# sjulier/Refactored_ORB_SLAM2

Measured on AMD Instinct MI355X. Metric: frames/s (extract+match) at KITTI 1241×376, 2000 feat; 1/2/4/8 GPU + CPU ref, higher is better.
Workload: dtype u8; 1 GPU; kitti_stereo_1241x376_2000feat_8lvl: 2x ORBextractor + ComputeStereoMatches + SearchByProjection(cur,last); parallelism=frame-shard x1, collective=none, driver=torch, queries=one pass: orbfe_track_queries_stereo_device

## Files before the change

refactored_orb_slam2_amd/csrc/match_kernels.hip:

```cpp
#include <string.h>
#include <atomic>
#include <mutex>

#include "match_internal.h"

#define WAVE 64

__device__ __forceinline__ int hamming256(const uint4 a0, const uint4 a1, const uint4 b0, const uint4 b1) {
  return __popc(a0.x ^ b0.x) + __popc(a0.y ^ b0.y) + __popc(a0.z ^ b0.z) + __popc(a0.w ^ b0.w) +
         __popc(a1.x ^ b1.x) + __popc(a1.y ^ b1.y) + __popc(a1.z ^ b1.z) + __popc(a1.w ^ b1.w);
}
__device__ __forceinline__ void load_desc(const uint8_t* p, uint4& d0, uint4& d1) {
  const uint4* q = reinterpret_cast<const uint4*>(p);
  d0 = q[0];
  d1 = q[1];
}
__device__ __forceinline__ void load_desc4(const uint8_t* p, uint4& d0, uint4& d1) {
  const uint32_t* q = reinterpret_cast<const uint32_t*>(p);
  d0 = make_uint4(q[0], q[1], q[2], q[3]);
  d1 = make_uint4(q[4], q[5], q[6], q[7]);
}

__device__ __forceinline__ unsigned wave_min_u32(unsigned v) {
#define ORBFE_MIN_STEP(ctrl, rmask) v = min(v, (unsigned)__builtin_amdgcn_update_dpp((int)0xffffffff, (int)v, ctrl, rmask, 0xf, false))
// ... 837 lines not shown
  for (int i = lane; i < pr.countB; i += WAVE)
    taken[i] = (uint8_t)((P.sequential && __hip_atomic_load(&P.matchB[P.idxB[pr.startB + i]], __ATOMIC_RELAXED, __HIP_MEMORY_SCOPE_AGENT) >= 0) ||
                         (P.validB && !P.validB[P.idxB[pr.startB + i]]));
  __syncthreads();
  for (int iKF = 0; iKF < pr.countA; iKF++) {
    const int realIdxKF = P.idxA[pr.startA + iKF];
    if (!P.validA[realIdxKF]) continue;
    uint4 a0, a1;
    load_desc(P.descA + (size_t)realIdxKF * 32, a0, a1);
    int bestd = 256, bestj = -1, second = 256;
    for (int iF = lane; iF < pr.countB; iF += WAVE) {
      if (taken[iF]) continue;
      const int realIdxF = P.idxB[pr.startB + iF];
      uint4 b0, b1;
      load_desc(P.descB + (size_t)realIdxF * 32, b0, b1);
      const int d = hamming256(a0, a1, b0, b1);
      if (d < bestd) { second = bestd; bestd = d; bestj = iF; }
      else if (d < second) second = d;
    }
    const unsigned key = bestj >= 0 ? (((unsigned)bestd << 16) | (unsigned)bestj) : 0xFFFFFFFFu;
    const unsigned b = wave_min_u32(key);
    if (b != 0xFFFFFFFFu) {
      const unsigned other = (key == b) ? 0xFFFFFFFFu : key;
      int s2 = min(second, other != 0xFFFFFFFFu ? (int)(other >> 16) : 256);
#pragma unroll
      for (int d = 32; d >= 1; d >>= 1) s2 = min(s2, __shfl_xor(s2, d, WAVE));
      const int bestDist1 = (int)(b >> 16), bestF = (int)(b & 0xffff);
      if ((P.kf_mode ? bestDist1 < ORBFE_TH_LOW : bestDist1 <= ORBFE_TH_LOW) && (float)bestDist1 < P.nnratio * (float)s2) {
        if (lane == 0) {
          const int realIdxF = P.idxB[pr.startB + bestF];
          __hip_atomic_store(&P.matchB[realIdxF], realIdxKF, __ATOMIC_RELAXED, __HIP_MEMORY_SCOPE_AGENT);
          if (P.kf_mode) P.matchA[realIdxKF] = realIdxF;
          taken[bestF] = 1;
          if (P.sequential)
            for (int t = 0; t < pr.countB; t++)
              if (P.idxB[pr.startB + t] == realIdxF) taken[t] = 1;
          if (P.check_ori) {
            float rot = P.angleA[realIdxKF] - P.angleB[realIdxF];
            if (rot < 0.0f) rot += 360.0f;
            int bin = (int)roundf(rot * (1.0f / ORBFE_HISTO_LENGTH));
            if (bin == ORBFE_HISTO_LENGTH) bin = 0;
            const int pos = atomicAdd(&P.counters[0], 1);
            P.push_idx[pos] = P.kf_mode ? realIdxKF : realIdxF;
            P.push_bin[pos] = (uint8_t)bin;
            atomicAdd(&P.counters[2 + bin], 1);
          }
          atomicAdd(&P.counters[1], 1);
        }
      }
    }
    __syncthreads();
  }
  }
}

__global__ __launch_bounds__(64) void triangulation_match_kernel(TriParams T) {
  const BowParams& P = T.b;
  const int lane = threadIdx.x;
  const int first = P.sequential ? 0 : blockIdx.x, last = P.sequential ? P.n_pairs : blockIdx.x + 1;
  for (int pi = first; pi < last; pi++) {
    const BowPair pr = P.pairs[pi];
    for (int i1 = 0; i1 < pr.countA; i1++) {
      const int idx1 = P.idxA[pr.startA + i1];
      if (!P.validA[idx1]) continue;
      const bool bStereo1 = T.stereoA[idx1] != 0;
      const orbfe_keypoint kp1 = T.keysA[idx1];
      uint4 a0, a1;
      load_desc(P.descA + (size_t)idx1 * 32, a0, a1);
      const float* F = T.ep.F12;
      const float la = kp1.x * F[0] + kp1.y * F[3] + F[6];
      const float lb = kp1.x * F[1] + kp1.y * F[4] + F[7];
      const float lc = kp1.x * F[2] + kp1.y * F[5] + F[8];
      const float den = la * la + lb * lb;
      unsigned key = 0xFFFFFFFFu;
      for (int i2 = lane; i2 < pr.countB; i2 += WAVE) {
        const int idx2 = P.idxB[pr.startB + i2];
        if (!P.validB[idx2]) continue;
        uint4 b0, b1;
        load_desc(P.descB + (size_t)idx2 * 32, b0, b1);
        const int dist = hamming256(a0, a1, b0, b1);
        if (dist > ORBFE_TH_LOW) continue;
        const orbfe_keypoint kp2 = T.keysB[idx2];
        if (!bStereo1 && !T.stereoB[idx2]) {
          const float distex = T.ep.ex - kp2.x, distey = T.ep.ey - kp2.y;
          if (distex * distex + distey * distey < 100 * T.ep.scale_factors[kp2.octave & (ORBFE_MAX_LEVELS - 1)]) continue;
        }
        const float num = la * kp2.x + lb * kp2.y + lc;
        if (den == 0) continue;
        const float dsqr = num * num / den;
        if (!((double)dsqr < 3.84 * (double)T.ep.level_sigma2[kp2.octave & (ORBFE_MAX_LEVELS - 1)])) continue;
        const unsigned k = ((unsigned)dist << 16) | (unsigned)(0xffff - i2);
        key = min(key, k);
      }
      const unsigned b = wave_min_u32(key);
      if (b != 0xFFFFFFFFu && lane == 0) {
        const int idx2 = P.idxB[pr.startB + (0xffff - (int)(b & 0xffff))];
        P.matchA[idx1] = idx2;
        atomicAdd(&P.counters[1], 1);
        if (P.check_ori) {
          float rot = kp1.angle - T.keysB[idx2].angle;
          if (rot < 0.0f) rot += 360.0f;
          int bin = (int)roundf(rot * (1.0f / ORBFE_HISTO_LENGTH));
          if (bin == ORBFE_HISTO_LENGTH) bin = 0;
          const int pos = atomicAdd(&P.counters[0], 1);
          P.push_idx[pos] = idx1;
          P.push_bin[pos] = (uint8_t)bin;
          atomicAdd(&P.counters[2 + bin], 1);
        }
      }
    }
  }
}

__global__ __launch_bounds__(256) void bow_finish_kernel(BowParams P) {
  __shared__ int top[3];
  __shared__ int removed;
  if (threadIdx.x == 0) {
    removed = 0;
    int i1, i2, i3;
    three_maxima(P.counters + 2, ORBFE_HISTO_LENGTH, i1, i2, i3);
    top[0] = i1; top[1] = i2; top[2] = i3;
  }
  __syncthreads();
  if (P.check_ori) {
    const int np = P.counters[0];
    int r = 0;
    for (int k = threadIdx.x; k < np; k += 256) {
      const int bin = P.push_bin[k];
      if (bin != top[0] && bin != top[1] && bin != top[2]) { (P.kf_mode ? P.matchA : P.matchB)[P.push_idx[k]] = -1; r++; }
    }
    if (r) atomicAdd(&removed, r);
  }
  __syncthreads();
  if (threadIdx.x == 0) P.counters[1] -= removed;
}

__global__ __launch_bounds__(64) void init_resolve_kernel(FrameBatch F, QueryBatch Q, const orbfe_cand* __restrict__ cand,
                                                           const int32_t* __restrict__ n_cand, int max_cand, float nnratio,
                                                           int check_ori, int32_t* __restrict__ matches12,
                                                           float* __restrict__ prev_xy, int32_t* __restrict__ n_matches,
                                                           int32_t* __restrict__ push_idx, uint8_t* __restrict__ push_bin) {
  __shared__ int hist[ORBFE_HISTO_LENGTH];
  extern __shared__ __attribute__((aligned(16))) uint8_t dyn[];
  int* matchedDist = reinterpret_cast<int*>(dyn);
  int* matches21 = matchedDist + F.cap;
  const int lane = threadIdx.x;
  const int n1 = Q.n[0], n2 = F.n[0];
  const orbfe_keypoint* keys2 = F.keys;
  for (int i = lane; i < n2; i += WAVE) { matchedDist[i] = 2147483647; matches21[i] = -1; }
  for (int i = lane; i < n1; i += WAVE) matches12[i] = -1;
  if (lane < ORBFE_HISTO_LENGTH) hist[lane] = 0;
  __syncthreads();
  int npush = 0;
  for (int i1 = 0; i1 < n1; i1++) {
    const orbfe_query* qp = Q.q + i1;
    if (!qp->valid) continue;
    const int total = n_cand[i1];
    if (total == 0) continue;
    unsigned k1 = 0xFFFFFFFFu, k2 = 0xFFFFFFFFu;
    int i1b = -1;
    auto consider = [&](int rank, int idx, int dist, int = 0) {
      if (matchedDist[idx] <= dist) return;
      const unsigned key = ((unsigned)dist << 16) | (unsigned)min(rank, 0xffff);
      if (key < k1) { k2 = k1; k1 = key; i1b = idx; }
      else if (key < k2) { k2 = key; }
    };
    if (total <= max_cand) {
      const orbfe_cand* cl = cand + (size_t)i1 * max_cand;
      for (int c = lane; c < total; c += WAVE) consider(c, cl[c].idx, cl[c].dist & 0xffff, 0);
    } else {
      const orbfe_query q = *qp;
      uint4 d0, d1;
      load_desc4(qp->desc, d0, d1);
      enumerate_window(F, 0, q, d0, d1, consider);
    }
    const unsigned b = wave_min_u32(k1);
    if (b != 0xFFFFFFFFu) {
      const unsigned long long wm = __ballot(k1 == b);
      const int wl = __ffsll((long long)wm) - 1;
      const int bestIdx2 = __builtin_amdgcn_readlane(i1b, wl);
      const int bestDist = (int)(b >> 16);
      const unsigned mine = (lane == wl) ? k2 : k1;
      const unsigned s2 = wave_min_u32(mine);
      const int bestDist2 = s2 != 0xFFFFFFFFu ? (int)(s2 >> 16) : 2147483647;
      if (bestDist <= ORBFE_TH_LOW && (float)bestDist < (float)bestDist2 * nnratio) {
        if (lane == 0) {
          const int prev = matches21[bestIdx2];
          if (prev >= 0) matches12[prev] = -1;
          matches12[i1] = bestIdx2;
          matches21[bestIdx2] = i1;
          matchedDist[bestIdx2] = bestDist;
          if (check_ori) {
            float rot = qp->angle - keys2[bestIdx2].angle;
            if (rot < 0.0f) rot += 360.0f;
            int bin = (int)roundf(rot * (1.0f / ORBFE_HISTO_LENGTH));
            if (bin == ORBFE_HISTO_LENGTH) bin = 0;
            push_idx[npush] = i1;
            push_bin[npush] = (uint8_t)bin;
            hist[bin]++;
          }
        }
        npush += check_ori ? 1 : 0;
      }
    }
    __syncthreads();
  }
  __syncthreads();
  if (lane == 0) {
    if (check_ori) {
      int a, b2, c;
      three_maxima(hist, ORBFE_HISTO_LENGTH, a, b2, c);
      for (int k = 0; k < npush; k++) {
        const int bin = push_bin[k];
        if (bin != a && bin != b2 && bin != c) {
          const int idx1 = push_idx[k];
          if (matches12[idx1] >= 0) matches12[idx1] = -1;
        }
      }
    }
  }
  __syncthreads();
  int cnt = 0;
  for (int i = lane; i < n1; i += WAVE) {
    const int m = matches12[i];
    if (m >= 0) {
      cnt++;
      prev_xy[2 * i] = keys2[m].x;
      prev_xy[2 * i + 1] = keys2[m].y;
    }
  }
  cnt = wave_sum_i32(cnt);
  if (lane == 0) n_matches[0] = cnt;
}

__global__ __launch_bounds__(256) void stereo_bucket_kernel(StereoParams P) {
  extern __shared__ int sb_lds[];
  int* cnt = sb_lds;
  int* start = sb_lds + P.n_keys;
  __shared__ int part[256];
  const int pair = blockIdx.x, tid = threadIdx.x;
  const int nR = P.nR[pair];
  const int nb = P.n_buckets, nl = P.n_levels, nk = P.n_keys;
  const orbfe_keypoint* kr = P.kpsR + (size_t)pair * P.cap;
  int32_t* bs = P.bucket_start + (size_t)pair * (nk + 1);
  int4* bi = reinterpret_cast<int4*>(P.bucket_idx) + (size_t)pair * P.cap * STEREO_BUCKET_SPAN;
  for (int b = tid; b < nk; b += 256) cnt[b] = 0;
  __syncthreads();
  for (int pass = 0; pass < 2; pass++) {
    for (int iR = tid; iR < nR; iR += 256) {
      const orbfe_keypoint kp = kr[iR];
      const int oct = min(max(kp.octave, 0), nl - 1);
      const float r = 2.0f * P.scale[oct];
      const int maxr = (int)ceilf(kp.y + r), minr = (int)floorf(kp.y - r);
      int b0 = max(minr, 0) >> 3, b1 = min(maxr >> 3, nb - 1);
      if (b1 - b0 >= STEREO_BUCKET_SPAN) b1 = b0 + STEREO_BUCKET_SPAN - 1;
      for (int b = b0; b <= b1; b++) {
        const int key = b * nl + oct;
        const int pos = atomicAdd(&cnt[key], 1);
        if (pass == 1) bi[start[key] + pos] = make_int4(iR, __float_as_int(kp.x), __float_as_int(kp.y), kp.octave);
      }
    }
    __syncthreads();
    if (pass == 0) {
      const int per = (nk + 255) / 256;
      const int k0 = min(tid * per, nk), k1 = min(k0 + per, nk);
      int sum = 0;
      for (int k = k0; k < k1; k++) sum += cnt[k];
      part[tid] = sum;
      __syncthreads();
      if (tid == 0) {
        int run = 0;
        for (int i = 0; i < 256; i++) { const int v = part[i]; part[i] = run; run += v; }
        start[nk] = run;
      }
      __syncthreads();
      int run = part[tid];
      for (int k = k0; k < k1; k++) { start[k] = run; run += cnt[k]; }
      __syncthreads();
      for (int b = tid; b <= nk; b += 256) bs[b] = start[b];
      for (int b = tid; b < nk; b += 256) cnt[b] = 0;
      __syncthreads();
    }
  }
}

__device__ __forceinline__ unsigned sad_u32(unsigned a, unsigned b, unsigned c) {
  unsigned r;
  asm("v_sad_u32 %0, %1, %2, %3" : "=v"(r) : "v"(a), "v"(b), "v"(c));
  return r;
}
#define ORBFE_ROW_ALL(op, v) do { \
    v = op(v, (unsigned)__builtin_amdgcn_update_dpp(0, (int)v, 0x128, 0xf, 0xf, false));  \
    v = op(v, (unsigned)__builtin_amdgcn_update_dpp(0, (int)v, 0x124, 0xf, 0xf, false));  \
    v = op(v, (unsigned)__builtin_amdgcn_update_dpp(0, (int)v, 0x122, 0xf, 0xf, false));  \
    v = op(v, (unsigned)__builtin_amdgcn_update_dpp(0, (int)v, 0x121, 0xf, 0xf, false));  \
  } while (0)
__device__ __forceinline__ unsigned op_min_u(unsigned a, unsigned b) { return min(a, b); }
__device__ __forceinline__ unsigned op_add_u(unsigned a, unsigned b) { return a + b; }
__device__ __forceinline__ unsigned op_or_u(unsigned a, unsigned b) { return a | b; }
__device__ __forceinline__ unsigned row_min_u32(unsigned v) { ORBFE_ROW_ALL(op_min_u, v); return v; }
__device__ __forceinline__ unsigned row_sum_u32(unsigned v) { ORBFE_ROW_ALL(op_add_u, v); return v; }
__device__ __forceinline__ unsigned row_or_u32(unsigned v) { ORBFE_ROW_ALL(op_or_u, v); return v; }

struct SmLevel {
  const uint8_t* baseL; const uint8_t* baseR;
  unsigned long long strideL, strideR;
  int pitchL, pitchR, wL, hL, wR, hR;
  float scale, inv_scale;
  int tiledL, tiledR;
};
#define SM_G 16
#define SM_KPB (256 / SM_G)
#ifndef SM_ROUNDS
#define SM_ROUNDS 2
#endif
#ifndef SM_SAD_T
#define SM_SAD_T 8
#endif
#define SAD_LP 32
#define SAD_RP 48
#define SAD_WIN (11 * SAD_LP + 11 * SAD_RP + 16)
#ifndef SM_XCD_PAIRS
#define SM_XCD_PAIRS 1
#endif
__global__ __launch_bounds__(256) void stereo_match_kernel(StereoParams P) {
  int pair = blockIdx.y, bx = blockIdx.x;
#if SM_XCD_PAIRS
  {
    const unsigned gx = gridDim.x;
    const unsigned lin = blockIdx.y * gx + blockIdx.x;
    const unsigned g8 = lin / (8u * gx);
    if (8u * g8 + 8u <= gridDim.y) {
      const unsigned within = lin - g8 * 8u * gx;
      pair = (int)(8u * g8 + (within & 7u));
      bx = (int)(within >> 3);
    }
  }
#endif
  const int lane = threadIdx.x & (WAVE - 1);
  const int sub = lane & (SM_G - 1);
  const int grp = threadIdx.x / SM_G;
  const int iL = bx * SM_KPB + grp;
  __shared__ SmLevel s_lv[ORBFE_MAX_LEVELS];
  __shared__ float s_r[ORBFE_MAX_LEVELS];
  __shared__ __attribute__((aligned(16))) uint8_t sad_win[SM_KPB][SAD_WIN];
  __shared__ uint16_t s_offL[128], s_offR[128];
  if (threadIdx.x >= 128) {
    const unsigned p = threadIdx.x - 128, yy = p / 11u, xx = p - yy * 11u;
    s_offL[p] = (uint16_t)(p < 121 ? yy * SAD_LP + xx : 0);
    s_offR[p] = (uint16_t)(p < 121 ? yy * SAD_RP + xx : 0);
  }
  if (threadIdx.x < ORBFE_MAX_LEVELS) {
    const int l = threadIdx.x;
    const bool in = l < P.n_levels;
    SmLevel v;
    v.baseL = P.pyrL.base[l] + (size_t)pair * P.pyrL.img_stride[l];
    v.baseR = P.pyrR.base[l] + (size_t)pair * P.pyrR.img_stride[l];
    v.strideL = 0; v.strideR = 0;
    v.pitchL = P.pyrL.pitch[l]; v.pitchR = P.pyrR.pitch[l];
    v.wL = in ? P.pyrL.w[l] : 0; v.hL = in ? P.pyrL.h[l] : 0;
    v.wR = in ? P.pyrR.w[l] : 0; v.hR = in ? P.pyrR.h[l] : 0;
    v.scale = P.scale[l]; v.inv_scale = P.inv_scale[l];
    v.tiledL = (int)((P.pyrL.tiled >> l) & 1u); v.tiledR = (int)((P.pyrR.tiled >> l) & 1u);
    s_lv[l] = v;
    s_r[l] = 2.0f * P.scale[l];
  }
  __syncthreads();
  const int cap = P.cap, nl = P.n_levels;
  float* out_ur = P.u_right + (size_t)pair * cap;
  float* out_depth = P.depth + (size_t)pair * cap;
  int32_t* out_sad = P.sad + (size_t)pair * cap;
  const orbfe_keypoint* kl = P.kpsL + (size_t)pair * cap;
  const uint8_t* dl = P.descL + (size_t)pair * cap * 32;
  const uint8_t* dr = P.descR + (size_t)pair * cap * 32;
  const int nL = P.nL[pair];
  const int iLc = min(iL, cap - 1);
  const float uL = kl[iLc].x, vL = kl[iLc].y;
  const int octL = kl[iLc].octave;
  uint4 a0, a1;
  load_desc(dl + (size_t)iLc * 32, a0, a1);
  if (sub == 0 && iL < cap) { out_ur[iL] = -1.0f; out_depth[iL] = -1.0f; out_sad[iL] = -1; }
  const int levelL = min(max(octL, 0), nl - 1);
  const int nRows = P.pyrL.h[0];
  const int row = (int)vL;
  const float minD = 0, maxD = P.maxD;
  const float minU = uL - maxD, maxU = uL - minD;
  bool act = iL < nL && row >= 0 && row < nRows && !(maxU < 0);
  const int32_t* bs = P.bucket_start + (size_t)pair * (P.n_keys + 1);
  const int4* bent = reinterpret_cast<const int4*>(P.bucket_idx) + (size_t)pair * cap * STEREO_BUCKET_SPAN;
  const int kb = act ? (row >> 3) * nl : 0;
  const int e0 = bs[kb + max(levelL - 1, 0)];
  const int e1 = act ? bs[kb + min(levelL + 1, nl - 1) + 1] : e0;
  unsigned best = ((unsigned)ORBFE_TH_HIGH << 16) | 0xffffu;
  float best_x = 0.f;
  const float rowm1 = (float)(row - 1), rowp1 = (float)(row + 1);
  for (int eb = e0; __ballot(eb < e1) != 0ull; eb += SM_ROUNDS * SM_G) {
    int4 rec[SM_ROUNDS];
    bool ok[SM_ROUNDS];
    float rx[SM_ROUNDS];
#pragma unroll
    for (int r = 0; r < SM_ROUNDS; r++) {
      const int e = eb + r * SM_G + sub;
      ok[r] = e < e1;
      rec[r] = bent[max(min(e, e1 - 1), 0)];
    }
    uint4 b0[SM_ROUNDS], b1[SM_ROUNDS];
#pragma unroll
    for (int r = 0; r < SM_ROUNDS; r++) {
      rx[r] = __int_as_float(rec[r].y);
      const float ry = __int_as_float(rec[r].z);
      const float rad = s_r[rec[r].w & (ORBFE_MAX_LEVELS - 1)];
      ok[r] = ok[r] && (ry + rad > rowm1) && (ry - rad < rowp1) && (rx[r] >= minU && rx[r] <= maxU);
      load_desc(dr + (size_t)(ok[r] ? rec[r].x : 0) * 32, b0[r], b1[r]);
    }
#pragma unroll
    for (int r = 0; r < SM_ROUNDS; r++) {
      if (__ballot(ok[r]) != 0ull) {
        const unsigned key = ((unsigned)hamming256(a0, a1, b0[r], b1[r]) << 16) | (unsigned)rec[r].x;
        if (ok[r] && key < best) {
          best = key;
          best_x = rx[r];
        }
      }
    }
  }
  {
    const unsigned k = ((best >> 16) < (unsigned)ORBFE_TH_HIGH) ? best : 0xFFFFFFFFu;
    best = row_min_u32(k);
    best_x = __int_as_float((int)row_or_u32((k == best && k != 0xFFFFFFFFu) ? (unsigned)__float_as_int(best_x) : 0u));
  }
  const float uR0 = best_x;
  const int thOrbDist = (ORBFE_TH_HIGH + ORBFE_TH_LOW) / 2;
  act = act && best != 0xFFFFFFFFu && (int)(best >> 16) < thOrbDist;
  if (__ballot(act) == 0ull) return;

  const SmLevel lv = s_lv[levelL];
  const float sfac = lv.inv_scale;
  const float scaleduL = roundf(uL * sfac);
  const float scaledvL = roundf(vL * sfac);
  const float scaleduR0 = roundf(uR0 * sfac);
  const int w = 5, L = 5;
  const float iniu = scaleduR0 + L - w;
  const float endu = scaleduR0 + L + w + 1;
  act = act && !(iniu < 0 || endu >= (float)lv.wR);
  const int yW = (int)(scaledvL - w), xW = (int)(scaleduL - w), xRc = (int)scaleduR0;
  const int xR0 = xRc - L - w;
  act = act && !(yW < 0 || yW + 2 * w >= lv.hL || xW < 0 || xW + 2 * w >= lv.wL || xR0 < 0 || xRc + L + w >= lv.wR ||
                 yW + 2 * w >= lv.hR);
  if (__ballot(act) == 0ull) return;
  uint8_t* winL = &sad_win[grp][0];
  uint8_t* winR = winL + 11 * SAD_LP;
  const int axL = xW & ~15, axR = xR0 & ~15;
  if (act && sub < 11) {
    typedef const __attribute__((address_space(1))) uint8_t* gptr_t;
    typedef unsigned int u32x4 __attribute__((ext_vector_type(4)));
    const int y = yW + sub;
    u32x4 vl[2], vr[3];
#pragma unroll
    for (int k = 0; k < 2; k++) {
      const int x = min(axL + 16 * k, lv.pitchL - 16);
      vl[k] = *reinterpret_cast<const __attribute__((address_space(1))) u32x4*>((gptr_t)(uintptr_t)lv.baseL + orbfe_level_offset(x, y, lv.pitchL, lv.tiledL != 0));
    }
#pragma unroll
    for (int k = 0; k < 3; k++) {
      const int x = min(axR + 16 * k, lv.pitchR - 16);
      vr[k] = *reinterpret_cast<const __attribute__((address_space(1))) u32x4*>((gptr_t)(uintptr_t)lv.baseR + orbfe_level_offset(x, y, lv.pitchR, lv.tiledR != 0));
    }
    u32x4* wl = reinterpret_cast<u32x4*>(winL + sub * SAD_LP);
    wl[0] = vl[0]; wl[1] = vl[1];
    u32x4* wr = reinterpret_cast<u32x4*>(winR + sub * SAD_RP);
    wr[0] = vr[0]; wr[1] = vr[1]; wr[2] = vr[2];
  }
  __builtin_amdgcn_fence(__ATOMIC_RELEASE, "wavefront");
  __builtin_amdgcn_wave_barrier();
  __builtin_amdgcn_fence(__ATOMIC_ACQUIRE, "wavefront");
  const uint8_t* WL = winL + (xW - axL);
  const uint8_t* WR = winR + (xR0 - axR);
  const int cLm = (int)WL[w * SAD_LP + w] - 255;
  int cRm[11];
#pragma unroll
  for (int k = 0; k < 11; k++) cRm[k] = (int)WR[w * SAD_RP + w + k] - 255;
  unsigned acc[11];
#pragma unroll
  for (int k = 0; k < 11; k++) acc[k] = 0;
#pragma unroll
  for (int t = 0; t < SM_SAD_T; t++) {
    const int p = sub + SM_G * t;
    if (t < 7 || p < 121) {
      const unsigned a = (unsigned)((int)WL[s_offL[p]] - cLm);
      const uint8_t* rrow = WR + s_offR[p];
#pragma unroll
      for (int k = 0; k < 11; k++) acc[k] = sad_u32(a, (unsigned)((int)rrow[k] - cRm[k]), acc[k]);
    }
  }
  unsigned pk[6];
#pragma unroll
  for (int j = 0; j < 5; j++) pk[j] = acc[2 * j] | (acc[2 * j + 1] << 16);
  pk[5] = acc[10];
#pragma unroll
  for (int j = 0; j < 6; j++) pk[j] = row_sum_u32(pk[j]);
  unsigned mine = pk[0];
  {
    const int t = sub >> 1;
    mine = t == 1 ? pk[1] : mine; mine = t == 2 ? pk[2] : mine; mine = t == 3 ? pk[3] : mine;
    mine = t == 4 ? pk[4] : mine; mine = t == 5 ? pk[5] : mine;
    mine = (sub & 1) ? (mine >> 16) : (mine & 0xffffu);
  }
  const unsigned kmin = row_min_u32(sub < 11 ? ((mine << 4) | (unsigned)sub) : 0xFFFFFFFFu);
  const int bk = (int)(kmin & 15u);
  const int sadBest = (int)(kmin >> 4);
  const int bestincR = bk - L;
  const int rowbase = lane & ~(SM_G - 1);
  const int i1 = __builtin_amdgcn_ds_bpermute((rowbase + ((bk + 15) & 15)) << 2, (int)mine);
  const int i3 = __builtin_amdgcn_ds_bpermute((rowbase + ((bk + 1) & 15)) << 2, (int)mine);
  const int i2 = sadBest;
  if (!act || sub != 0 || bestincR == -L || bestincR == L) return;
  const float dist1 = (float)i1, dist2 = (float)i2, dist3 = (float)i3;
  const float deltaR = (dist1 - dist3) / (2.0f * (dist1 + dist3 - 2.0f * dist2));
  if (deltaR < -1 || deltaR > 1) return;
  float bestuR = lv.scale * ((float)scaleduR0 + (float)bestincR + deltaR);
  float disparity = (uL - bestuR);
  if (disparity >= minD && disparity < maxD) {
    if (disparity <= 0) {
      disparity = (float)0.01;
      bestuR = (float)((double)uL - 0.01);
    }
    out_depth[iL] = P.mbf / disparity;
    out_ur[iL] = bestuR;
    out_sad[iL] = sadBest;
  }
}

__global__ __launch_bounds__(256) void stereo_median_kernel(StereoParams P) {
  __shared__ int hist[256];
  __shared__ int sh[4];
  const int pair = blockIdx.x, tid = threadIdx.x;
  const int nL = P.nL[pair];
  float* out_ur = P.u_right + (size_t)pair * P.cap;
  float* out_depth = P.depth + (size_t)pair * P.cap;
  const int32_t* sad = P.sad + (size_t)pair * P.cap;
  hist[tid] = 0;
  if (tid == 0) sh[0] = 0;
  __syncthreads();
  int cntv = 0;
  for (int i = tid; i < nL; i += 256) {
    const int s = sad[i];
    if (s >= 0) { atomicAdd(&hist[(s >> 8) & 0xff], 1); cntv++; }
  }
  atomicAdd(&sh[0], cntv);
  __syncthreads();
  const int total = sh[0];
  if (total == 0) { if (tid == 0) P.n_matched[pair] = 0; return; }
  const int k = total / 2;
  if (tid == 0) {
    int run = 0, hb = 0;
    for (; hb < 256; hb++) { if (run + hist[hb] > k) break; run += hist[hb]; }
    sh[1] = hb;
    sh[2] = k - run;
  }
  __syncthreads();
  const int hb = sh[1], k2 = sh[2];
  __syncthreads();
  hist[tid] = 0;
  __syncthreads();
  for (int i = tid; i < nL; i += 256) {
    const int s = sad[i];
    if (s >= 0 && ((s >> 8) & 0xff) == hb) atomicAdd(&hist[s & 0xff], 1);
  }
  __syncthreads();
  if (tid == 0) {
    int run = 0, lb = 0;
    for (; lb < 256; lb++) { if (run + hist[lb] > k2) break; run += hist[lb]; }
    sh[3] = (hb << 8) | lb;
    sh[0] = 0;
  }
  __syncthreads();
  const float median = (float)sh[3];
  const float thDist = 1.5f * 1.4f * median;
  int kept = 0;
  for (int i = tid; i < nL; i += 256) {
    const int s = sad[i];
    if (s >= 0) {
      if ((float)s < thDist) kept++;
      else { out_ur[i] = -1; out_depth[i] = -1; }
    }
  }
  atomicAdd(&sh[0], kept);
  __syncthreads();
  if (tid == 0) P.n_matched[pair] = sh[0];
}

static void raise_dynamic_lds(const void* kernel, int bytes, std::atomic<unsigned long long>& done) {
  int dev = 0;
  if (hipGetDevice(&dev) != hipSuccess) dev = 0;
  const unsigned long long bit = 1ull << (dev & 63);
  if (done.load(std::memory_order_acquire) & bit) return;
  (void)hipFuncSetAttribute(kernel, hipFuncAttributeMaxDynamicSharedMemorySize, bytes);
  done.fetch_or(bit, std::memory_order_release);
}
void orbfe_launch_hamming_matrix(const uint8_t* A, int nA, const uint8_t* B, int nB, uint16_t* out, hipStream_t s) {
  if (nA < 1 || nB < 1) return;
  dim3 grid((nB + 255) / 256, (nA + 63) / 64);
  hipLaunchKernelGGL(hamming_matrix_kernel, grid, dim3(256), 0, s, A, nA, B, nB, out);
}
void orbfe_launch_hamming_bf(const HammingBfParams& p, int max_nA, int n_sets, hipStream_t s) {
  if (max_nA < 1 || n_sets < 1) return;
  dim3 grid((max_nA + 255) / 256, n_sets);
  hipLaunchKernelGGL(hamming_bf_kernel, grid, dim3(256), 0, s, p);
}
void orbfe_launch_grid_build(const FrameBatch& f, int n_frames, hipStream_t s) {
  if (f.cap > GB_LDS_CAP) {
    hipLaunchKernelGGL(grid_build_global_kernel, dim3(n_frames), dim3(GB_THREADS), 0, s, f);
    return;
  }
  static std::atomic<unsigned long long> raised{0};
  raise_dynamic_lds(reinterpret_cast<const void*>(grid_build_kernel), 6 * GB_LDS_CAP + 16, raised);
  hipLaunchKernelGGL(grid_build_kernel, dim3(n_frames), dim3(GB_THREADS), (size_t)6 * (size_t)f.cap + 16, s, f);
}
void orbfe_launch_proj_candidates(const FrameBatch& f, const QueryBatch& q, orbfe_cand* cand, int32_t* n_cand,
                                  int max_cand, int n_frames, hipStream_t s) {
  if (q.cap < 1) return;
  constexpr int G = ORBFE_CAND_LANES;
  dim3 grid((q.cap + 4 * (64 / G) - 1) / (4 * (64 / G)), n_frames);
  hipLaunchKernelGGL(proj_candidates_kernel<G>, grid, dim3(256), 0, s, f, q, cand, n_cand, max_cand);
}
void orbfe_launch_proj_resolve(const FrameBatch& f, const QueryBatch& q, const orbfe_cand* cand, const int32_t* n_cand,
                               int max_cand, int mode, int th_high, float nnratio, int check_ori, uint8_t* blocked,
                               int32_t* assigned, int32_t* n_matches, int32_t* push_idx, uint8_t* push_bin, int n_frames,
                               hipStream_t s) {
  const size_t dyn = (size_t)(((f.cap + 15) & ~15) + 8 * (size_t)f.cap);
  static std::atomic<unsigned long long> raised{0};
  raise_dynamic_lds(reinterpret_cast<const void*>(proj_resolve_kernel), 88 * 1024, raised);
  hipLaunchKernelGGL(proj_resolve_kernel, dim3(n_frames), dim3(RC_THREADS), dyn, s, f, q, cand, n_cand, max_cand, mode, th_high,
                     nnratio, check_ori, blocked, assigned, n_matches, push_idx, push_bin);
}
void orbfe_launch_bow(const BowParams& p, int n_pairs, int max_countB, hipStream_t s) {
  if (n_pairs > 0)
    hipLaunchKernelGGL(bow_match_kernel, dim3(p.sequential ? 1 : n_pairs), dim3(64), (size_t)((max_countB + 15) & ~15), s, p);
  hipLaunchKernelGGL(bow_finish_kernel, dim3(1), dim3(256), 0, s, p);
}
void orbfe_launch_proj_best(const FrameBatch& f, const QueryBatch& q, int gate, const float* inv_sigma2, int32_t* best_idx,
                            int32_t* best_dist, int n_frames, hipStream_t s) {
  if (q.cap < 1) return;
  dim3 grid((q.cap + 3) / 4, n_frames);
  if (gate == 2) hipLaunchKernelGGL(proj_best_kernel<2>, grid, dim3(256), 0, s, f, q, inv_sigma2, best_idx, best_dist);
  else if (gate == 1) hipLaunchKernelGGL(proj_best_kernel<1>, grid, dim3(256), 0, s, f, q, inv_sigma2, best_idx, best_dist);
  else hipLaunchKernelGGL(proj_best_kernel<0>, grid, dim3(256), 0, s, f, q, inv_sigma2, best_idx, best_dist);
}
void orbfe_launch_triangulation(const TriParams& p, int n_pairs, hipStream_t s) {
  if (n_pairs > 0) hipLaunchKernelGGL(triangulation_match_kernel, dim3(p.b.sequential ? 1 : n_pairs), dim3(64), 0, s, p);
  hipLaunchKernelGGL(bow_finish_kernel, dim3(1), dim3(256), 0, s, p.b);
}
void orbfe_launch_init_resolve(const FrameBatch& f, const QueryBatch& q, const orbfe_cand* cand, const int32_t* n_cand,
                               int max_cand, float nnratio, int check_ori, int32_t* matches12, float* prev_xy,
                               int32_t* n_matches, int32_t* push_idx, uint8_t* push_bin, hipStream_t s) {
  hipLaunchKernelGGL(init_resolve_kernel, dim3(1), dim3(64), (size_t)f.cap * 8, s, f, q, cand, n_cand, max_cand, nnratio,
                     check_ori, matches12, prev_xy, n_matches, push_idx, push_bin);
}
void orbfe_launch_stereo(const StereoParams& p, int n_pairs, hipStream_t s) {
  const size_t bucket_lds = sizeof(int) * (size_t)(2 * p.n_keys + 1);
  if (bucket_lds > 48 * 1024) {
    static std::atomic<unsigned long long> raised{0};
    raise_dynamic_lds(reinterpret_cast<const void*>(stereo_bucket_kernel), (int)(sizeof(int) * (2 * STEREO_MAX_KEYS + 1)), raised);
  }
  hipLaunchKernelGGL(stereo_bucket_kernel, dim3(n_pairs), dim3(256), bucket_lds, s, p);
  dim3 grid((p.cap + SM_KPB - 1) / SM_KPB, n_pairs);
  hipLaunchKernelGGL(stereo_match_kernel, grid, dim3(256), 0, s, p);
  hipLaunchKernelGGL(stereo_median_kernel, dim3(n_pairs), dim3(256), 0, s, p);
}
```

Measured before the change: 113,800 frames/s.

## Trim stereo match kernel address math and precompute SAD offsets in constant memory

```diff
diff --git a/refactored_orb_slam2_amd/csrc/match_kernels.hip b/refactored_orb_slam2_amd/csrc/match_kernels.hip
--- a/refactored_orb_slam2_amd/csrc/match_kernels.hip
+++ b/refactored_orb_slam2_amd/csrc/match_kernels.hip
@@ -1163,13 +1163,6 @@
 __device__ __forceinline__ unsigned row_sum_u32(unsigned v) { ORBFE_ROW_ALL(op_add_u, v); return v; }
 __device__ __forceinline__ unsigned row_or_u32(unsigned v) { ORBFE_ROW_ALL(op_or_u, v); return v; }
 
-struct SmLevel {
-  const uint8_t* baseL; const uint8_t* baseR;
-  unsigned long long strideL, strideR;
-  int pitchL, pitchR, wL, hL, wR, hR;
-  float scale, inv_scale;
-  int tiledL, tiledR;
-};
 #define SM_G 16
 #define SM_KPB (256 / SM_G)
 #ifndef SM_ROUNDS
@@ -1181,6 +1174,28 @@
 #define SAD_LP 32
 #define SAD_RP 48
 #define SAD_WIN (11 * SAD_LP + 11 * SAD_RP + 16)
+struct StereoOffsets { uint16_t l[SM_G][8], r[SM_G][8]; };
+static constexpr StereoOffsets make_stereo_offsets() {
+  StereoOffsets T{};
+  for (int sub = 0; sub < SM_G; sub++)
+    for (int t = 0; t < 8; t++) {
+      const int p = sub + SM_G * t, yy = p / 11, xx = p - yy * 11;
+      T.l[sub][t] = (uint16_t)(p < 121 ? yy * SAD_LP + xx : 0);
+      T.r[sub][t] = (uint16_t)(p < 121 ? yy * SAD_RP + xx : 0);
+    }
+  return T;
+}
+__constant__ __attribute__((aligned(16))) const StereoOffsets stereo_offsets = make_stereo_offsets();
+
+template <typename T>
+__device__ __forceinline__ T ld_at(const void* base, unsigned byte_off) {
+  return *reinterpret_cast<const T*>(static_cast<const uint8_t*>(base) + byte_off);
+}
+__device__ __forceinline__ unsigned lane_select(unsigned a, unsigned b, unsigned long long mask) {
+  unsigned r;
+  asm("v_cndmask_b32 %0, %1, %2, %3" : "=v"(r) : "v"(a), "v"(b), "s"(mask));
+  return r;
+}
 #ifndef SM_XCD_PAIRS
 #define SM_XCD_PAIRS 1
 #endif
@@ -1198,72 +1213,78 @@
     }
   }
 #endif
-  const int lane = threadIdx.x & (WAVE - 1);
-  const int sub = lane & (SM_G - 1);
-  const int grp = threadIdx.x / SM_G;
-  const int iL = bx * SM_KPB + grp;
-  __shared__ SmLevel s_lv[ORBFE_MAX_LEVELS];
+  size_t upair = (size_t)(unsigned)pair;
+  asm("" : "+s"(upair));
+  const unsigned lane = threadIdx.x & (WAVE - 1);
+  const unsigned sub = lane & (SM_G - 1);
+  const unsigned grp = threadIdx.x / SM_G;
+  const int iL = bx * SM_KPB + (int)grp;
+  __shared__ uint4 s_lv[ORBFE_MAX_LEVELS][4];
   __shared__ float s_r[ORBFE_MAX_LEVELS];
+  __shared__ float s_scale[ORBFE_MAX_LEVELS];
   __shared__ __attribute__((aligned(16))) uint8_t sad_win[SM_KPB][SAD_WIN];
-  __shared__ uint16_t s_offL[128], s_offR[128];
-  if (threadIdx.x >= 128) {
-    const unsigned p = threadIdx.x - 128, yy = p / 11u, xx = p - yy * 11u;
-    s_offL[p] = (uint16_t)(p < 121 ? yy * SAD_LP + xx : 0);
-    s_offR[p] = (uint16_t)(p < 121 ? yy * SAD_RP + xx : 0);
-  }
   if (threadIdx.x < ORBFE_MAX_LEVELS) {
     const int l = threadIdx.x;
     const bool in = l < P.n_levels;
-    SmLevel v;
-    v.baseL = P.pyrL.base[l] + (size_t)pair * P.pyrL.img_stride[l];
-    v.baseR = P.pyrR.base[l] + (size_t)pair * P.pyrR.img_stride[l];
-    v.strideL = 0; v.strideR = 0;
-    v.pitchL = P.pyrL.pitch[l]; v.pitchR = P.pyrR.pitch[l];
-    v.wL = in ? P.pyrL.w[l] : 0; v.hL = in ? P.pyrL.h[l] : 0;
-    v.wR = in ? P.pyrR.w[l] : 0; v.hR = in ? P.pyrR.h[l] : 0;
-    v.scale = P.scale[l]; v.inv_scale = P.inv_scale[l];
-    v.tiledL = (int)((P.pyrL.tiled >> l) & 1u); v.tiledR = (int)((P.pyrR.tiled >> l) & 1u);
-    s_lv[l] = v;
+    const unsigned long long bL = (unsigned long long)(uintptr_t)(P.pyrL.base[l] + upair * P.pyrL.img_stride[l]);
+    const unsigned long long bR = (unsigned long long)(uintptr_t)(P.pyrR.base[l] + upair * P.pyrR.img_stride[l]);
+    const int pitchL = P.pyrL.pitch[l], pitchR = P.pyrR.pitch[l];
+    const int wL = in ? P.pyrL.w[l] : 0, hL = in ? P.pyrL.h[l] : 0, wR = in ? P.pyrR.w[l] : 0, hR = in ? P.pyrR.h[l] : 0;
+    const bool tL = (P.pyrL.tiled >> l) & 1u, tR = (P.pyrR.tiled >> l) & 1u;
+    s_lv[l][0] = make_uint4((unsigned)__float_as_int(P.inv_scale[l]), (unsigned)max(min(hL, hR) - 10, 0), (unsigned)max(wL - 10, 0),
+                            (unsigned)max(wR - 21, 0));
+    s_lv[l][1] = make_uint4(8u * pitchL, tL ? 16u : (unsigned)pitchL, tL ? 128u : 16u, (unsigned)((pitchL >> 4) - 1));
+    s_lv[l][2] = make_uint4(8u * pitchR, tR ? 16u : (unsigned)pitchR, tR ? 128u : 16u, (unsigned)((pitchR >> 4) - 1));
+    s_lv[l][3] = make_uint4((unsigned)bL, (unsigned)(bL >> 32), (unsigned)bR, (unsigned)(bR >> 32));
     s_r[l] = 2.0f * P.scale[l];
+    s_scale[l] = P.scale[l];
   }
   __syncthreads();
   const int cap = P.cap, nl = P.n_levels;
-  float* out_ur = P.u_right + (size_t)pair * cap;
-  float* out_depth = P.depth + (size_t)pair * cap;
-  int32_t* out_sad = P.sad + (size_t)pair * cap;
-  const orbfe_keypoint* kl = P.kpsL + (size_t)pair * cap;
-  const uint8_t* dl = P.descL + (size_t)pair * cap * 32;
-  const uint8_t* dr = P.descR + (size_t)pair * cap * 32;
-  const int nL = P.nL[pair];
-  const int iLc = min(iL, cap - 1);
-  const float uL = kl[iLc].x, vL = kl[iLc].y;
-  const int octL = kl[iLc].octave;
-  uint4 a0, a1;
-  load_desc(dl + (size_t)iLc * 32, a0, a1);
-  if (sub == 0 && iL < cap) { out_ur[iL] = -1.0f; out_depth[iL] = -1.0f; out_sad[iL] = -1; }
+  float* out_ur = P.u_right + upair * cap;
+  float* out_depth = P.depth + upair * cap;
+  int32_t* out_sad = P.sad + upair * cap;
+  const orbfe_keypoint* kl = P.kpsL + upair * cap;
+  const uint8_t* dl = P.descL + upair * cap * 32;
+  const uint8_t* dr = P.descR + upair * cap * 32;
+  const int nL = P.nL[upair];
+  const unsigned iLc = (unsigned)min(iL, cap - 1);
+  const unsigned kofs = __umul24(iLc, (unsigned)sizeof(orbfe_keypoint));
+  const float2 uvL = ld_at<float2>(kl, kofs);
+  const float uL = uvL.x, vL = uvL.y;
+  const int octL = ld_at<int>(kl, kofs + (unsigned)offsetof(orbfe_keypoint, octave));
+  const uint4 a0 = ld_at<uint4>(dl, iLc * 32u), a1 = ld_at<uint4>(dl, iLc * 32u + 16u);
+  const unsigned oofs = (unsigned)iL * 4u;
+  if (sub == 0 && iL < cap) {
+    *reinterpret_cast<float*>(reinterpret_cast<uint8_t*>(out_ur) + oofs) = -1.0f;
+    *reinterpret_cast<float*>(reinterpret_cast<uint8_t*>(out_depth) + oofs) = -1.0f;
+    *reinterpret_cast<int32_t*>(reinterpret_cast<uint8_t*>(out_sad) + oofs) = -1;
+  }
   const int levelL = min(max(octL, 0), nl - 1);
   const int nRows = P.pyrL.h[0];
   const int row = (int)vL;
   const float minD = 0, maxD = P.maxD;
   const float minU = uL - maxD, maxU = uL - minD;
   bool act = iL < nL && row >= 0 && row < nRows && !(maxU < 0);
-  const int32_t* bs = P.bucket_start + (size_t)pair * (P.n_keys + 1);
-  const int4* bent = reinterpret_cast<const int4*>(P.bucket_idx) + (size_t)pair * cap * STEREO_BUCKET_SPAN;
-  const int kb = act ? (row >> 3) * nl : 0;
-  const int e0 = bs[kb + max(levelL - 1, 0)];
-  const int e1 = act ? bs[kb + min(levelL + 1, nl - 1) + 1] : e0;
+  const int32_t* bs = P.bucket_start + upair * (P.n_keys + 1);
+  const int4* bent = reinterpret_cast<const int4*>(P.bucket_idx) + upair * cap * STEREO_BUCKET_SPAN;
+  const int kb = act ? (int)__umul24((unsigned)row >> 3, (unsigned)nl) : 0;
+  const int e0 = ld_at<int>(bs, (unsigned)(kb + max(levelL - 1, 0)) * 4u);
+  const int e1r = ld_at<int>(bs, (unsigned)(kb + min(levelL + 1, nl - 1)) * 4u + 4u);
+  const int e1 = act ? e1r : e0;
   unsigned best = ((unsigned)ORBFE_TH_HIGH << 16) | 0xffffu;
   float best_x = 0.f;
   const float rowm1 = (float)(row - 1), rowp1 = (float)(row + 1);
-  for (int eb = e0; __ballot(eb < e1) != 0ull; eb += SM_ROUNDS * SM_G) {
+  const int e1s = e1 + (int)sub, e1m = max(e1 - 1, 0);
+  for (int eb = e0 + (int)sub; __ballot(eb < e1s) != 0ull; eb += SM_ROUNDS * SM_G) {
     int4 rec[SM_ROUNDS];
     bool ok[SM_ROUNDS];
     float rx[SM_ROUNDS];
 #pragma unroll
     for (int r = 0; r < SM_ROUNDS; r++) {
-      const int e = eb + r * SM_G + sub;
+      const int e = eb + r * SM_G;
       ok[r] = e < e1;
-      rec[r] = bent[max(min(e, e1 - 1), 0)];
+      rec[r] = ld_at<int4>(bent, (unsigned)min(e, e1m) << 4);
     }
     uint4 b0[SM_ROUNDS], b1[SM_ROUNDS];
 #pragma unroll
@@ -1272,7 +1293,9 @@
       const float ry = __int_as_float(rec[r].z);
       const float rad = s_r[rec[r].w & (ORBFE_MAX_LEVELS - 1)];
       ok[r] = ok[r] && (ry + rad > rowm1) && (ry - rad < rowp1) && (rx[r] >= minU && rx[r] <= maxU);
-      load_desc(dr + (size_t)(ok[r] ? rec[r].x : 0) * 32, b0[r], b1[r]);
+      const unsigned dofs = (unsigned)(ok[r] ? rec[r].x : 0) * 32u;
+      b0[r] = ld_at<uint4>(dr, dofs);
+      b1[r] = ld_at<uint4>(dr, dofs + 16u);
     }
 #pragma unroll
     for (int r = 0; r < SM_ROUNDS; r++) {
@@ -1295,48 +1318,49 @@
   act = act && best != 0xFFFFFFFFu && (int)(best >> 16) < thOrbDist;
   if (__ballot(act) == 0ull) return;
 
-  const SmLevel lv = s_lv[levelL];
-  const float sfac = lv.inv_scale;
+  const uint4 lvb = s_lv[levelL][0];
+  const float sfac = __int_as_float((int)lvb.x);
   const float scaleduL = roundf(uL * sfac);
   const float scaledvL = roundf(vL * sfac);
   const float scaleduR0 = roundf(uR0 * sfac);
   const int w = 5, L = 5;
-  const float iniu = scaleduR0 + L - w;
-  const float endu = scaleduR0 + L + w + 1;
-  act = act && !(iniu < 0 || endu >= (float)lv.wR);
   const int yW = (int)(scaledvL - w), xW = (int)(scaleduL - w), xRc = (int)scaleduR0;
   const int xR0 = xRc - L - w;
-  act = act && !(yW < 0 || yW + 2 * w >= lv.hL || xW < 0 || xW + 2 * w >= lv.wL || xR0 < 0 || xRc + L + w >= lv.wR ||
-                 yW + 2 * w >= lv.hR);
+  act = act && (unsigned)yW < lvb.y && (unsigned)xW < lvb.z && (unsigned)xR0 < lvb.w;
   if (__ballot(act) == 0ull) return;
-  uint8_t* winL = &sad_win[grp][0];
-  uint8_t* winR = winL + 11 * SAD_LP;
-  const int axL = xW & ~15, axR = xR0 & ~15;
+  const unsigned winL = (unsigned)(uintptr_t)&sad_win[0][0] + grp * SAD_WIN;
+  const unsigned winR = winL + 11 * SAD_LP;
+  const uint4 offL = *reinterpret_cast<const uint4*>(&stereo_offsets.l[sub][0]);
+  const uint4 offR = *reinterpret_cast<const uint4*>(&stereo_offsets.r[sub][0]);
   if (act && sub < 11) {
+    typedef unsigned int u32x4 __attribute__((ext_vector_type(4)));
     typedef const __attribute__((address_space(1))) uint8_t* gptr_t;
-    typedef unsigned int u32x4 __attribute__((ext_vector_type(4)));
-    const int y = yW + sub;
+    typedef const __attribute__((address_space(1))) u32x4* gvec_t;
+    const uint4 gL = s_lv[levelL][1], gR = s_lv[levelL][2], gB = s_lv[levelL][3];
+    const gptr_t pL = (gptr_t)(uintptr_t)(((unsigned long long)gB.y << 32) | gB.x);
+    const gptr_t pR = (gptr_t)(uintptr_t)(((unsigned long long)gB.w << 32) | gB.z);
+    const unsigned y = (unsigned)yW + sub, yh = y >> 3, yl = y & 7u;
+    const unsigned rowL = __umul24(yh, gL.x) + __umul24(yl, gL.y);
+    const unsigned rowR = __umul24(yh, gR.x) + __umul24(yl, gR.y);
+    const unsigned cL = (unsigned)xW >> 4, cR = (unsigned)xR0 >> 4;
     u32x4 vl[2], vr[3];
-#pragma unroll
-    for (int k = 0; k < 2; k++) {
-      const int x = min(axL + 16 * k, lv.pitchL - 16);
-      vl[k] = *reinterpret_cast<const __attribute__((address_space(1))) u32x4*>((gptr_t)(uintptr_t)lv.baseL + orbfe_level_offset(x, y, lv.pitchL, lv.tiledL != 0));
-    }
-#pragma unroll
-    for (int k = 0; k < 3; k++) {
-      const int x = min(axR + 16 * k, lv.pitchR - 16);
-      vr[k] = *reinterpret_cast<const __attribute__((address_space(1))) u32x4*>((gptr_t)(uintptr_t)lv.baseR + orbfe_level_offset(x, y, lv.pitchR, lv.tiledR != 0));
-    }
-    u32x4* wl = reinterpret_cast<u32x4*>(winL + sub * SAD_LP);
+    vl[0] = *(gvec_t)(pL + (rowL + __umul24(cL, gL.z)));
+    vl[1] = *(gvec_t)(pL + (rowL + __umul24(min(cL + 1u, gL.w), gL.z)));
+    vr[0] = *(gvec_t)(pR + (rowR + __umul24(cR, gR.z)));
+    vr[1] = *(gvec_t)(pR + (rowR + __umul24(min(cR + 1u, gR.w), gR.z)));
+    vr[2] = *(gvec_t)(pR + (rowR + __umul24(min(cR + 2u, gR.w), gR.z)));
+    typedef __attribute__((address_space(3))) u32x4* lvec_t;
+    lvec_t wl = (lvec_t)(uintptr_t)(winL + sub * SAD_LP);
     wl[0] = vl[0]; wl[1] = vl[1];
-    u32x4* wr = reinterpret_cast<u32x4*>(winR + sub * SAD_RP);
+    lvec_t wr = (lvec_t)(uintptr_t)(winR + sub * SAD_RP);
     wr[0] = vr[0]; wr[1] = vr[1]; wr[2] = vr[2];
   }
   __builtin_amdgcn_fence(__ATOMIC_RELEASE, "wavefront");
   __builtin_amdgcn_wave_barrier();
   __builtin_amdgcn_fence(__ATOMIC_ACQUIRE, "wavefront");
-  const uint8_t* WL = winL + (xW - axL);
-  const uint8_t* WR = winR + (xR0 - axR);
+  typedef const __attribute__((address_space(3))) uint8_t* lptr_t;
+  const lptr_t WL = (lptr_t)(uintptr_t)(winL + ((unsigned)xW & 15u));
+  const lptr_t WR = (lptr_t)(uintptr_t)(winR + ((unsigned)xR0 & 15u));
   const int cLm = (int)WL[w * SAD_LP + w] - 255;
   int cRm[11];
 #pragma unroll
@@ -1344,12 +1368,14 @@
   unsigned acc[11];
 #pragma unroll
   for (int k = 0; k < 11; k++) acc[k] = 0;
+  const unsigned oLw[4] = {offL.x, offL.y, offL.z, offL.w}, oRw[4] = {offR.x, offR.y, offR.z, offR.w};
 #pragma unroll
   for (int t = 0; t < SM_SAD_T; t++) {
-    const int p = sub + SM_G * t;
-    if (t < 7 || p < 121) {
-      const unsigned a = (unsigned)((int)WL[s_offL[p]] - cLm);
-      const uint8_t* rrow = WR + s_offR[p];
+    if (t < 7 || sub < 121 - SM_G * 7) {
+      const unsigned ol = (t & 1) ? (oLw[t >> 1] >> 16) : (oLw[t >> 1] & 0xffffu);
+      const unsigned orr = (t & 1) ? (oRw[t >> 1] >> 16) : (oRw[t >> 1] & 0xffffu);
+      const unsigned a = (unsigned)((int)WL[ol] - cLm);
+      const lptr_t rrow = WR + orr;
 #pragma unroll
       for (int k = 0; k < 11; k++) acc[k] = sad_u32(a, (unsigned)((int)rrow[k] - cRm[k]), acc[k]);
     }
@@ -1360,35 +1386,36 @@
   pk[5] = acc[10];
 #pragma unroll
   for (int j = 0; j < 6; j++) pk[j] = row_sum_u32(pk[j]);
-  unsigned mine = pk[0];
+  unsigned mine;
   {
-    const int t = sub >> 1;
-    mine = t == 1 ? pk[1] : mine; mine = t == 2 ? pk[2] : mine; mine = t == 3 ? pk[3] : mine;
-    mine = t == 4 ? pk[4] : mine; mine = t == 5 ? pk[5] : mine;
-    mine = (sub & 1) ? (mine >> 16) : (mine & 0xffffu);
-  }
-  const unsigned kmin = row_min_u32(sub < 11 ? ((mine << 4) | (unsigned)sub) : 0xFFFFFFFFu);
+    const unsigned m01 = lane_select(pk[0], pk[1], 0xCCCCCCCCCCCCCCCCull);
+    const unsigned m23 = lane_select(pk[2], pk[3], 0xCCCCCCCCCCCCCCCCull);
+    const unsigned m45 = lane_select(pk[4], pk[5], 0xCCCCCCCCCCCCCCCCull);
+    mine = lane_select(lane_select(m01, m23, 0xF0F0F0F0F0F0F0F0ull), m45, 0xFF00FF00FF00FF00ull);
+    mine = __builtin_amdgcn_ubfe(mine, (sub & 1u) << 4, 16);
+  }
+  const unsigned kmin = row_min_u32((mine << 4) | (sub < 11 ? sub : 0xFFFFFFFFu));
   const int bk = (int)(kmin & 15u);
   const int sadBest = (int)(kmin >> 4);
   const int bestincR = bk - L;
-  const int rowbase = lane & ~(SM_G - 1);
-  const int i1 = __builtin_amdgcn_ds_bpermute((rowbase + ((bk + 15) & 15)) << 2, (int)mine);
-  const int i3 = __builtin_amdgcn_ds_bpermute((rowbase + ((bk + 1) & 15)) << 2, (int)mine);
+  const unsigned rowbase4 = (lane & ~(unsigned)(SM_G - 1)) << 2;
+  const int i1 = __builtin_amdgcn_ds_bpermute((int)((((kmin << 2) + 60u) & 60u) | rowbase4), (int)mine);
+  const int i3 = __builtin_amdgcn_ds_bpermute((int)((((kmin << 2) + 4u) & 60u) | rowbase4), (int)mine);
   const int i2 = sadBest;
   if (!act || sub != 0 || bestincR == -L || bestincR == L) return;
   const float dist1 = (float)i1, dist2 = (float)i2, dist3 = (float)i3;
   const float deltaR = (dist1 - dist3) / (2.0f * (dist1 + dist3 - 2.0f * dist2));
   if (deltaR < -1 || deltaR > 1) return;
-  float bestuR = lv.scale * ((float)scaleduR0 + (float)bestincR + deltaR);
+  float bestuR = s_scale[levelL] * ((float)scaleduR0 + (float)bestincR + deltaR);
   float disparity = (uL - bestuR);
   if (disparity >= minD && disparity < maxD) {
     if (disparity <= 0) {
       disparity = (float)0.01;
       bestuR = (float)((double)uL - 0.01);
     }
-    out_depth[iL] = P.mbf / disparity;
-    out_ur[iL] = bestuR;
-    out_sad[iL] = sadBest;
+    *reinterpret_cast<float*>(reinterpret_cast<uint8_t*>(out_depth) + oofs) = P.mbf / disparity;
+    *reinterpret_cast<float*>(reinterpret_cast<uint8_t*>(out_ur) + oofs) = bestuR;
+    *reinterpret_cast<int32_t*>(reinterpret_cast<uint8_t*>(out_sad) + oofs) = sadBest;
   }
 }
 
```

Result: no change. 114,300 frames/s (median of 6 runs) (+0.4%).
